# martinsbruveris/tensorflow-image-models

Measured on NVIDIA H100. Metric: images/sec fwd bs=256 224px, higher is better.
Workload: dtype bf16

## Files before the change

tensorflow-image-models_b200/csrc/common.cuh:

```cuda
#pragma once

#include <cuda.h>
#include <cuda_bf16.h>
#include <cuda_runtime.h>
#include <stdint.h>
#include <stdio.h>

#include <atomic>

#include "tfimm_b200.h"

namespace tfimm {

enum Status : int {
  kOk = TFIMM_OK,
  kInvalidArgument = TFIMM_ERR_INVALID_ARGUMENT,
  kCudaError = TFIMM_ERR_CUDA,
  kUnsupported = TFIMM_ERR_UNSUPPORTED,
};

void set_last_error(const char* fmt, ...);
int cuda_fail(cudaError_t e, const char* what);

#define TFIMM_CHECK_ARG(cond, ...)                \
// ... 277 lines not shown
__device__ __forceinline__ void st8(__nv_bfloat16* p, const float (&v)[8]) {
  uint4 a;
  a.x = pack_bf16x2(v[0], v[1]);
  a.y = pack_bf16x2(v[2], v[3]);
  a.z = pack_bf16x2(v[4], v[5]);
  a.w = pack_bf16x2(v[6], v[7]);
  *reinterpret_cast<uint4*>(p) = a;
}

__device__ __forceinline__ uint32_t smem_u32(const void* p) {
  return static_cast<uint32_t>(__cvta_generic_to_shared(p));
}

__device__ __forceinline__ bool elect_one() {
  uint32_t pred = 0;
  asm volatile(
      "{\n"
      ".reg .pred P;\n"
      "elect.sync _|P, 0xffffffff;\n"
      "selp.u32 %0, 1, 0, P;\n"
      "}\n"
      : "=r"(pred));
  return pred != 0;
}

__device__ __forceinline__ void mbar_init(uint32_t bar, uint32_t count) {
  asm volatile("mbarrier.init.shared::cta.b64 [%0], %1;" ::"r"(bar), "r"(count) : "memory");
}
__device__ __forceinline__ void fence_mbar_init() {
  asm volatile("fence.mbarrier_init.release.cluster;" ::: "memory");
}
__device__ __forceinline__ void mbar_expect_tx(uint32_t bar, uint32_t bytes) {
  asm volatile("mbarrier.arrive.expect_tx.shared::cta.b64 _, [%0], %1;" ::"r"(bar), "r"(bytes)
               : "memory");
}
__device__ __forceinline__ void mbar_arrive(uint32_t bar) {
  asm volatile("mbarrier.arrive.shared::cta.b64 _, [%0];" ::"r"(bar) : "memory");
}
__device__ __forceinline__ bool mbar_try_wait(uint32_t bar, uint32_t parity) {
  uint32_t ok;
  asm volatile(
      "{\n"
      ".reg .pred P;\n"
#ifdef TFIMM_TRYWAIT_NO_HINT
      "mbarrier.try_wait.parity.shared::cta.b64 P, [%1], %2;\n"
#else
      "mbarrier.try_wait.parity.shared::cta.b64 P, [%1], %2, %3;\n"
#endif
      "selp.u32 %0, 1, 0, P;\n"
      "}\n"
      : "=r"(ok)
      : "r"(bar), "r"(parity), "r"(1000000u)
      : "memory");
  return ok != 0;
}
__device__ __forceinline__ void mbar_wait(uint32_t bar, uint32_t parity) {
  if (mbar_try_wait(bar, parity)) return;
  const long long t0 = clock64();
  uint32_t polls = 0;
  while (!mbar_try_wait(bar, parity)) {
    if ((++polls & 255u) == 0 && clock64() - t0 > 4000000000LL) __trap();
  }
}

__device__ __forceinline__ void fence_proxy_async_smem() {
  asm volatile("fence.proxy.async.shared::cta;" ::: "memory");
}

template <int kId>
__device__ __forceinline__ void named_bar_sync(int threads) {
  asm volatile("bar.sync %0, %1;" ::"n"(kId), "r"(threads) : "memory");
}

__device__ __forceinline__ void prefetch_tmap(const void* tmap) {
  asm volatile("prefetch.tensormap [%0];" ::"l"(reinterpret_cast<uint64_t>(tmap)) : "memory");
}

__device__ __forceinline__ void tma_load_2d(uint32_t dst_smem, const void* tmap, uint32_t bar,
                                            int c0, int c1) {
  asm volatile(
      "cp.async.bulk.tensor.2d.shared::cluster.global.mbarrier::complete_tx::bytes"
      " [%0], [%1, {%3, %4}], [%2];"
      ::"r"(dst_smem), "l"(reinterpret_cast<uint64_t>(tmap)), "r"(bar), "r"(c0), "r"(c1)
      : "memory");
}
__device__ __forceinline__ void tma_store_2d(const void* tmap, uint32_t src_smem, int c0, int c1) {
  asm volatile(
      "cp.async.bulk.tensor.2d.global.shared::cta.bulk_group [%0, {%2, %3}], [%1];"
      ::"l"(reinterpret_cast<uint64_t>(tmap)), "r"(src_smem), "r"(c0), "r"(c1)
      : "memory");
}
__device__ __forceinline__ void tma_load_3d(uint32_t dst_smem, const void* tmap, uint32_t bar, int c0,
                                            int c1, int c2) {
  asm volatile(
      "cp.async.bulk.tensor.3d.shared::cluster.global.mbarrier::complete_tx::bytes"
      " [%0], [%1, {%3, %4, %5}], [%2];"
      ::"r"(dst_smem), "l"(reinterpret_cast<uint64_t>(tmap)), "r"(bar), "r"(c0), "r"(c1), "r"(c2)
      : "memory");
}
__device__ __forceinline__ void tma_load_4d(uint32_t dst_smem, const void* tmap, uint32_t bar, int c0,
                                            int c1, int c2, int c3) {
  asm volatile(
      "cp.async.bulk.tensor.4d.shared::cluster.global.mbarrier::complete_tx::bytes"
      " [%0], [%1, {%3, %4, %5, %6}], [%2];"
      ::"r"(dst_smem), "l"(reinterpret_cast<uint64_t>(tmap)), "r"(bar), "r"(c0), "r"(c1), "r"(c2), "r"(c3)
      : "memory");
}
__device__ __forceinline__ void tma_store_4d(const void* tmap, uint32_t src_smem, int c0, int c1, int c2, int c3) {
  asm volatile(
      "cp.async.bulk.tensor.4d.global.shared::cta.bulk_group [%0, {%2, %3, %4, %5}], [%1];"
      ::"l"(reinterpret_cast<uint64_t>(tmap)), "r"(src_smem), "r"(c0), "r"(c1), "r"(c2), "r"(c3)
      : "memory");
}
__device__ __forceinline__ void tma_store_3d(const void* tmap, uint32_t src_smem, int c0, int c1, int c2) {
  asm volatile(
      "cp.async.bulk.tensor.3d.global.shared::cta.bulk_group [%0, {%2, %3, %4}], [%1];"
      ::"l"(reinterpret_cast<uint64_t>(tmap)), "r"(src_smem), "r"(c0), "r"(c1), "r"(c2)
      : "memory");
}
__device__ __forceinline__ void tma_store_commit() {
  asm volatile("cp.async.bulk.commit_group;" ::: "memory");
}
template <int N>
__device__ __forceinline__ void tma_store_wait_read() {
  asm volatile("cp.async.bulk.wait_group.read %0;" ::"n"(N) : "memory");
}
template <int N>
__device__ __forceinline__ void tma_store_wait_all() {
  asm volatile("cp.async.bulk.wait_group %0;" ::"n"(N) : "memory");
}

__device__ __forceinline__ uint64_t gmma_desc_k_sw128(uint32_t smem_addr) {
  uint64_t d = 0;
  d |= (uint64_t)((smem_addr >> 4) & 0x3FFF);
  d |= (uint64_t)1 << 16;
  d |= (uint64_t)(1024 >> 4) << 32;
  d |= (uint64_t)1 << 62;
  return d;
}
__device__ __forceinline__ uint64_t gmma_desc_mn_sw128(uint32_t smem_addr) {
  uint64_t d = 0;
  d |= (uint64_t)((smem_addr >> 4) & 0x3FFF);
  d |= (uint64_t)(8192 >> 4) << 16;
  d |= (uint64_t)(1024 >> 4) << 32;
  d |= (uint64_t)1 << 62;
  return d;
}
__device__ __forceinline__ void cluster_arrive_release() {
  asm volatile("barrier.cluster.arrive.release.aligned;" ::: "memory");
}
__device__ __forceinline__ void cluster_wait_acquire() {
  asm volatile("barrier.cluster.wait.acquire.aligned;" ::: "memory");
}

__device__ __forceinline__ void wgmma_fence() { asm volatile("wgmma.fence.sync.aligned;" ::: "memory"); }
__device__ __forceinline__ void wgmma_commit() { asm volatile("wgmma.commit_group.sync.aligned;" ::: "memory"); }
template <int N>
__device__ __forceinline__ void wgmma_wait() {
  asm volatile("wgmma.wait_group.sync.aligned %0;" ::"n"(N) : "memory");
}

__device__ __forceinline__ void cp_async_16(uint32_t dst_smem, const void* src, bool valid) {
  const int sz = valid ? 16 : 0;
  asm volatile("cp.async.cg.shared.global [%0], [%1], 16, %2;" ::"r"(dst_smem), "l"(src), "r"(sz)
               : "memory");
}
__device__ __forceinline__ void cp_async_commit() { asm volatile("cp.async.commit_group;" ::: "memory"); }
template <int N>
__device__ __forceinline__ void cp_async_wait() {
  asm volatile("cp.async.wait_group %0;" ::"n"(N) : "memory");
}
__device__ __forceinline__ void ldmatrix_x4(uint32_t addr, uint32_t& r0, uint32_t& r1, uint32_t& r2,
                                            uint32_t& r3) {
  asm volatile("ldmatrix.sync.aligned.m8n8.x4.shared.b16 {%0, %1, %2, %3}, [%4];"
               : "=r"(r0), "=r"(r1), "=r"(r2), "=r"(r3)
               : "r"(addr));
}
__device__ __forceinline__ void ldmatrix_x4_trans(uint32_t addr, uint32_t& r0, uint32_t& r1,
                                                  uint32_t& r2, uint32_t& r3) {
  asm volatile("ldmatrix.sync.aligned.m8n8.x4.trans.shared.b16 {%0, %1, %2, %3}, [%4];"
               : "=r"(r0), "=r"(r1), "=r"(r2), "=r"(r3)
               : "r"(addr));
}
__device__ __forceinline__ void mma_bf16_16816(float (&d)[4], const uint32_t (&a)[4], uint32_t b0,
                                               uint32_t b1) {
  asm volatile(
      "mma.sync.aligned.m16n8k16.row.col.f32.bf16.bf16.f32 "
      "{%0, %1, %2, %3}, {%4, %5, %6, %7}, {%8, %9}, {%0, %1, %2, %3};"
      : "+f"(d[0]), "+f"(d[1]), "+f"(d[2]), "+f"(d[3])
      : "r"(a[0]), "r"(a[1]), "r"(a[2]), "r"(a[3]), "r"(b0), "r"(b1));
}

__device__ __forceinline__ uint32_t tf32_rna(float x) {
  uint32_t r;
  asm("cvt.rna.tf32.f32 %0, %1;" : "=r"(r) : "f"(x));
  return r;
}
__device__ __forceinline__ void mma_tf32_1688(float (&d)[4], const uint32_t (&a)[4], uint32_t b0, uint32_t b1) {
  asm volatile(
      "mma.sync.aligned.m16n8k8.row.col.f32.tf32.tf32.f32 "
      "{%0, %1, %2, %3}, {%4, %5, %6, %7}, {%8, %9}, {%0, %1, %2, %3};"
      : "+f"(d[0]), "+f"(d[1]), "+f"(d[2]), "+f"(d[3])
      : "r"(a[0]), "r"(a[1]), "r"(a[2]), "r"(a[3]), "r"(b0), "r"(b1));
}

#endif

}
```

tensorflow-image-models_b200/csrc/gemm_sm90.cu:

```cuda
#include <type_traits>

#include "gemm_epilogue.cuh"
#include "wgmma.cuh"

namespace tfimm {

namespace {

constexpr int kBlockM = 128;
constexpr int kRowBytes = 128;
constexpr int kConsumerThreads = 256;
constexpr int kProducerWarp = kConsumerThreads / 32;
constexpr int kNumGateWarps = 4;

enum ATransform : int {
  kANone = 0,
  kAGate = 1,
  kATf32 = 2,
};
enum GemmMode : int { kModeGemm = 0, kModeToken = 1, kModeGluCols = 2 };

template <int AX>
using OperandT = std::conditional_t<AX == kATf32, float, __nv_bfloat16>;
template <int AX>
// ... 249 lines not shown
    else if constexpr (MODE == kModeGluCols) epilogue_glu_cols<OutT, BLOCK_N>(p, acc, m_blk, n_blk, wg * 64);
    else if constexpr (STAGED)
      epilogue_staged<OutT, BLOCK_N>(p, acc, m_blk, n_blk, wg, smem_out, s_bias, s_gamma, res_bar, &tmap_c);
    else epilogue_frag<OutT, BLOCK_N>(p, acc, m_blk, n_blk, wg * 64);
  }
}

struct PersistentCfg {
  static constexpr int kBlockN = 256;
  static constexpr int kABytes = kBlockM * kRowBytes;
  static constexpr int kStageBytes = kABytes + kBlockN * kRowBytes;
  static constexpr int kStages = 3;
  static constexpr int kBoxes = 4;
  static constexpr int kOutBytes = 2 * kBoxes * kStagedBoxBytes;
  static constexpr int kVecBytes = 2 * 2 * kBlockN * 4;
  static constexpr int kNumBarriers = 2 * kStages + 2;
  static constexpr int kSmemBytes = kStages * kStageBytes + kOutBytes + kVecBytes + kNumBarriers * 8 + 1024;
};

template <typename OutT>
__global__ void __launch_bounds__(kConsumerThreads + 32, 1)
gemm_persistent_kernel(const __grid_constant__ CUtensorMap tmap_a, const __grid_constant__ CUtensorMap tmap_b,
                       const __grid_constant__ CUtensorMap tmap_c, const __grid_constant__ CUtensorMap tmap_r,
                       const GemmParams p) {
  using Cfg = PersistentCfg;
  constexpr int BN = Cfg::kBlockN, kStages = Cfg::kStages, kBlockK = 64;
  constexpr int kCols = staged_chunk_cols<OutT>(), kSpan = Cfg::kBoxes * kCols;

  extern __shared__ uint8_t smem_raw[];
  const uint32_t smem_tiles = (smem_u32(smem_raw) + 1023u) & ~1023u;
  const uint32_t smem_out = smem_tiles + kStages * Cfg::kStageBytes;
  const uint32_t smem_vec = smem_out + Cfg::kOutBytes;
  const uint32_t smem_bars = smem_vec + Cfg::kVecBytes;
  auto full_bar = [&](int s) { return smem_bars + 8u * s; };
  auto empty_bar = [&](int s) { return smem_bars + 8u * (kStages + s); };
  float* const s_vec = reinterpret_cast<float*>(smem_raw + (smem_vec - smem_u32(smem_raw)));

  const int warp_idx = threadIdx.x >> 5;
  const int lane = threadIdx.x & 31;
  if (warp_idx == kProducerWarp && lane == 0) {
    prefetch_tmap(&tmap_a);
    prefetch_tmap(&tmap_b);
    prefetch_tmap(&tmap_c);
    if (p.has_res) prefetch_tmap(&tmap_r);
    for (int s = 0; s < kStages; ++s) {
      mbar_init(full_bar(s), 1);
      mbar_init(empty_bar(s), 2);
    }
    mbar_init(smem_bars + 8u * (2 * kStages), 1);
    mbar_init(smem_bars + 8u * (2 * kStages + 1), 1);
    fence_mbar_init();
  }
  __syncthreads();

  const int num_n_tiles = (p.N + BN - 1) / BN;
  const int tiles = ((p.M + kBlockM - 1) / kBlockM) * num_n_tiles;
  const int num_k_blocks = (p.K + kBlockK - 1) / kBlockK;

  if (warp_idx == kProducerWarp) {
    if (threadIdx.x == kProducerWarp * 32) {
      int stage = 0;
      uint32_t phase = 0;
      for (int t = blockIdx.x; t < tiles; t += gridDim.x) {
        const int m_blk = t / num_n_tiles, n_blk = t % num_n_tiles;
        for (int kb = 0; kb < num_k_blocks; ++kb) {
          mbar_wait(empty_bar(stage), phase ^ 1u);
          const uint32_t sa = smem_tiles + stage * Cfg::kStageBytes;
          mbar_expect_tx(full_bar(stage), Cfg::kStageBytes);
          tma_load_2d(sa, &tmap_a, full_bar(stage), kb * kBlockK, m_blk * kBlockM);
          tma_load_2d(sa + Cfg::kABytes, &tmap_b, full_bar(stage), kb * kBlockK, n_blk * BN);
          if (++stage == kStages) { stage = 0; phase ^= 1u; }
        }
      }
    }
    return;
  }

  const int wg = warp_idx >> 2;
  const bool leader = (threadIdx.x & 127) == 0;
  const uint32_t s_wg = smem_out + (uint32_t)(wg * Cfg::kBoxes * kStagedBoxBytes);
  const uint32_t res_bar = smem_bars + 8u * (2 * kStages + wg);
  int stage = 0, prev = 0, buf = 0;
  uint32_t phase = 0, res_phase = 0;
  for (int t = blockIdx.x; t < tiles; t += gridDim.x, buf ^= 1) {
    const int m_blk = t / num_n_tiles, n_blk = t % num_n_tiles;
    const int row0 = m_blk * kBlockM + wg * 64;
    auto has_res_span = [&](int h) { return p.has_res && row0 < p.M && n_blk * BN + h * kSpan < p.N; };
    auto load_res_span = [&](int h) {
      const int col0 = n_blk * BN + h * kSpan, chunks = min(Cfg::kBoxes, (p.N - col0 + kCols - 1) / kCols);
      mbar_expect_tx(res_bar, (uint32_t)(chunks * kStagedBoxBytes));
      for (int ch = 0; ch < chunks; ++ch)
        tma_load_2d(s_wg + (uint32_t)(ch * kStagedBoxBytes), &tmap_r, res_bar, col0 + ch * kCols, row0);
    };
    float* const s_bias = s_vec + buf * 2 * BN;
    float* const s_gamma = s_bias + BN;
    const int n_own = n_blk * BN + threadIdx.x;
    const float bias_own = p.bias != nullptr && n_own < p.N ? __ldg(p.bias + n_own) : 0.f;
    const float gamma_own = p.gamma != nullptr && n_own < p.N ? __ldg(p.gamma + n_own) : 1.f;
    float acc[BN / 2];
#pragma unroll
    for (int i = 0; i < BN / 2; ++i) acc[i] = 0.f;
    for (int kb = 0; kb < num_k_blocks; ++kb) {
      mbar_wait(full_bar(stage), phase);
      const uint32_t sa = smem_tiles + stage * Cfg::kStageBytes;
      const uint64_t da = gmma_desc_k_sw128(sa + (uint32_t)wg * (64 * 128));
      const uint64_t db = gmma_desc_k_sw128(sa + Cfg::kABytes);
      wgmma_fence();
#pragma unroll
      for (int k = 0; k < 4; ++k)
        wgmma_ss<BN, false>(acc, da + (uint64_t)(2 * k), db + (uint64_t)(2 * k), (uint32_t)((kb | k) != 0));
      wgmma_commit();
      if (kb == 0) {
        s_bias[threadIdx.x] = bias_own;
        s_gamma[threadIdx.x] = gamma_own;
      }
      if (kb == num_k_blocks / 2 && leader) {
        tma_store_wait_read<0>();
        if (has_res_span(0)) load_res_span(0);
      }
      wgmma_wait<1>();
      if (kb > 0 && leader) mbar_arrive(empty_bar(prev));
      prev = stage;
      if (++stage == kStages) { stage = 0; phase ^= 1u; }
    }
    wgmma_wait<0>();
    if (leader) mbar_arrive(empty_bar(prev));

    named_bar_sync<1>(256);
    auto span = [&](auto h_const) {
      constexpr int h = decltype(h_const)::value;
      if (n_blk * BN + h * kSpan >= p.N) return;
      if constexpr (h > 0) {
        if (leader) {
          tma_store_wait_read<0>();
          if (has_res_span(h)) load_res_span(h);
        }
        warpgroup_bar_sync(wg);
      }
      if (has_res_span(h)) {
        mbar_wait(res_bar, res_phase);
        res_phase ^= 1u;
      }
      staged_apply<OutT, BN, h * kSpan, kSpan>(p, acc, s_wg, s_bias, s_gamma);
      fence_proxy_async_smem();
      warpgroup_bar_sync(wg);
      if (leader && row0 < p.M) staged_store<OutT, Cfg::kBoxes>(p, &tmap_c, s_wg, row0, n_blk * BN + h * kSpan);
    };
    span(std::integral_constant<int, 0>{});
    if constexpr (kSpan < BN) span(std::integral_constant<int, 1>{});
  }
  if (leader) tma_store_wait_read<0>();
}

int check_out(const void* C, long ldc, const void* residual, long ldr, int esize) {
  TFIMM_CHECK_ARG((reinterpret_cast<uintptr_t>(C) & 15u) == 0 && (ldc * esize) % 16 == 0,
                  "gemm: C must be 16-byte aligned with a row stride of a multiple of 16 bytes");
  TFIMM_CHECK_ARG(residual == nullptr || ((reinterpret_cast<uintptr_t>(residual) & 15u) == 0 && (ldr * esize) % 16 == 0),
                  "gemm: residual must be 16-byte aligned with a row stride of a multiple of 16 bytes");
  return kOk;
}

template <int BLOCK_N, typename OutT, int AX, int MODE, bool STAGED = false>
int launch_wgmma(const CUtensorMap& ta, const CUtensorMap& tb, const GemmParams& p, const char* what,
                 cudaStream_t stream, const CUtensorMap& tc = CUtensorMap{}, const CUtensorMap& tr = CUtensorMap{}) {
  using Cfg = GemmCfg<BLOCK_N, OutT, STAGED>;
  auto kernel = gemm_wgmma_kernel<BLOCK_N, OutT, AX, MODE, STAGED>;
  static std::atomic<unsigned long long> attr_devs{0};
  TFIMM_CUDA_OK(set_max_dynamic_smem(kernel, Cfg::kSmemBytes, attr_devs));
  const long imgs = MODE == kModeToken ? p.tk_imgs : 1;
  const long tiles = imgs * ((p.M + kBlockM - 1) / kBlockM) * ((p.N + BLOCK_N - 1) / BLOCK_N);
  kernel<<<(unsigned)tiles, gemm_threads<BLOCK_N, AX>(), Cfg::kSmemBytes, stream>>>(ta, tb, tc, tr, p);
  TFIMM_LAUNCH_OK(what);
  return kOk;
}

template <int kMaxN, typename F>
int with_block_n(int bn, const char* unsupported_fmt, F&& launch) {
  if constexpr (kMaxN >= 256) {
    if (bn == 256) return launch(std::integral_constant<int, 256>{});
  }
  if (bn == 128) return launch(std::integral_constant<int, 128>{});
  if (bn == 64) return launch(std::integral_constant<int, 64>{});
  set_last_error(unsupported_fmt, bn);
  return kInvalidArgument;
}

template <typename OutT>
int launch_persistent(const CUtensorMap& ta, const CUtensorMap& tb, const CUtensorMap& tc, const CUtensorMap& tr,
                      const GemmParams& p, cudaStream_t stream) {
  using Cfg = PersistentCfg;
  auto kernel = gemm_persistent_kernel<OutT>;
  static std::atomic<unsigned long long> attr_devs{0};
  TFIMM_CUDA_OK(set_max_dynamic_smem(kernel, Cfg::kSmemBytes, attr_devs));
  const long tiles = (long)((p.M + kBlockM - 1) / kBlockM) * ((p.N + Cfg::kBlockN - 1) / Cfg::kBlockN);
  const int grid = (int)std::min<long>(tiles, sm_count());
  kernel<<<grid, kConsumerThreads + 32, Cfg::kSmemBytes, stream>>>(ta, tb, tc, tr, p);
  TFIMM_LAUNCH_OK("gemm_persistent_kernel (bf16)");
  return kOk;
}

template <int BLOCK_N, typename OutT, int AX = kANone, int MODE = kModeGemm, bool PERSISTENT = false>
int launch_gemm(const void* A, int lda, const void* W, int ldw, const void* residual, int ldr, void* C, int ldc,
                GemmParams p, cudaStream_t stream) {
  static_assert(!PERSISTENT || (BLOCK_N == PersistentCfg::kBlockN && AX == kANone && MODE == kModeGemm),
                "the persistent instance is the plain bf16 GEMM at 256 columns");
  const int M = p.M, N = p.N, K = p.K;
  constexpr int kBlockK = block_k<AX>();
  CUtensorMap ta, tb;
  int st;
  if ((st = check_out(C, ldc, residual, ldr, (int)sizeof(OutT))) != kOk) return st;
  if ((st = make_tmap_2d(&ta, A, dtype_code<AX>(), M, K, lda, kBlockM, kBlockK, "A")) != kOk) return st;
  if ((st = make_tmap_2d(&tb, W, dtype_code<AX>(), N, K, ldw, BLOCK_N, kBlockK, "W")) != kOk) return st;
  p.c = C; p.res = residual; p.ldc = ldc; p.ldr = ldr;
  constexpr bool kStaged = AX == kANone && MODE == kModeGemm && (BLOCK_N <= 128 || PERSISTENT);
  if constexpr (kStaged) {
    if ((long)N * (long)sizeof(OutT) % 16 != 0)
      return launch_wgmma<BLOCK_N, OutT, AX, MODE>(ta, tb, p, "gemm_wgmma_kernel (bf16)", stream);
    constexpr int es = (int)sizeof(OutT), dt = es == 2 ? kBF16 : kF32;
    CUtensorMap tc, tr{};
    if ((st = make_tmap_2d(&tc, C, dt, M, N, ldc, 64, staged_chunk_cols<OutT>(), "C")) != kOk) return st;
    if (residual != nullptr &&
        (st = make_tmap_2d(&tr, residual, dt, M, N, ldr, 64, staged_chunk_cols<OutT>(), "residual")) != kOk)
      return st;
    if constexpr (PERSISTENT) return launch_persistent<OutT>(ta, tb, tc, tr, p, stream);
    else return launch_wgmma<BLOCK_N, OutT, AX, MODE, true>(ta, tb, p, "gemm_wgmma_kernel (bf16)", stream, tc, tr);
  }
  return launch_wgmma<BLOCK_N, OutT, AX, MODE>(
      ta, tb, p,
      AX == kATf32 ? "gemm_wgmma_kernel (tf32)"
                   : (MODE == kModeGluCols ? "gemm_wgmma_kernel (bf16 glu)" : "gemm_wgmma_kernel (bf16)"),
      stream);
}

template <int BLOCK_N, typename OutT>
int launch_token(const void* Wt, int ldw, const void* X, long ldx, long img_x, GemmParams p, cudaStream_t stream) {
  CUtensorMap ta, tb;
  int st;
  if ((st = check_out(p.c, p.ldc, p.res, p.ldr, (int)sizeof(OutT))) != kOk) return st;
  if ((st = make_tmap_2d(&ta, Wt, kBF16, p.M, p.K, ldw, kBlockM, 64, "token Wt")) != kOk) return st;
  {
    const uint64_t dims[3] = {(uint64_t)p.N, (uint64_t)p.K, (uint64_t)p.tk_imgs};
    const uint64_t strides[2] = {(uint64_t)ldx * 2, (uint64_t)img_x * 2};
    const uint32_t box[3] = {64u, 64u, 1u};
    if ((st = make_tmap(&tb, X, kBF16, 3, dims, strides, box, "token X")) != kOk) return st;
  }
  return launch_wgmma<BLOCK_N, OutT, kANone, kModeToken>(ta, tb, p, "gemm_wgmma_kernel (bf16 token mixing)", stream);
}

template <int BLOCK_N, typename OutT, int AX = kANone>
int launch_conv(const void* x, const void* W, int ldw, const void* residual, void* out, int B, int H, int Wd, int C,
                int Ho, int Wo, GemmParams p, cudaStream_t stream) {
  constexpr int kBlockK = block_k<AX>();
  constexpr uint64_t es = sizeof(OperandT<AX>);
  const int N = p.N, s = p.cv_stride;
  CUtensorMap ta, tb;
  int st;
  if ((st = check_out(out, N, residual, N, (int)sizeof(OutT))) != kOk) return st;
  {
    const uint64_t dims[4] = {(uint64_t)C, (uint64_t)Wd, (uint64_t)H, (uint64_t)B};
    const uint64_t strides[3] = {(uint64_t)C * es, (uint64_t)Wd * C * es, (uint64_t)H * Wd * C * es};
    const uint32_t box[4] = {(uint32_t)kBlockK, (uint32_t)(p.cv_pw * s), (uint32_t)(p.cv_ph * s), (uint32_t)p.cv_pb};
    const uint32_t estr[4] = {1u, (uint32_t)s, (uint32_t)s, 1u};
    if ((st = make_tmap(&ta, x, dtype_code<AX>(), 4, dims, strides, box, "conv input", 128, estr)) != kOk) return st;
  }
  if ((st = make_tmap_2d(&tb, W, dtype_code<AX>(), N, p.K, ldw, BLOCK_N, kBlockK, "conv weights")) != kOk) return st;
  p.c = out; p.res = residual; p.ldc = N; p.ldr = N;
  p.cv_B = B; p.cv_Ho = Ho; p.cv_Wo = Wo;
  return launch_wgmma<BLOCK_N, OutT, AX, kModeGemm>(
      ta, tb, p,
      AX == kATf32 ? "gemm_wgmma_kernel (tf32 implicit convolution)" : "gemm_wgmma_kernel (bf16 implicit convolution)",
      stream);
}

int pick_block_n(int M, int N) {
  const int sms = sm_count() > 0 ? sm_count() : 132;
  const int mt = (M + kBlockM - 1) / kBlockM;
  int best = 256;
  double best_cost = 1e30;
  for (int bn : {256, 128, 64}) {
    const int nt = (N + bn - 1) / bn;
    const long tiles = (long)mt * nt;
    const int slots = bn == 64 ? 2 * sms : sms;
    const long waves = (tiles + slots - 1) / slots;
    const double cost = (double)waves * (bn == 64 ? 2 * bn : bn) * (bn == 256 ? 1.0 : (bn == 128 ? 1.04 : 1.10));
    if (cost < best_cost) { best_cost = cost; best = bn; }
  }
  return best;
}

constexpr int kPersistent = 1;

int pick_block_n_bf16(int M, int N, int K, int out_dtype) {
  constexpr double kEpilogueK = 926.0, kPairWidth = 184.0;
  const int sms = sm_count() > 0 ? sm_count() : 132;
  const long mt = (M + kBlockM - 1) / kBlockM;
  if (N > 256 && (out_dtype == kF32 || N % 8 == 0) && mt * ((N + 255) / 256) >= sms) return kPersistent;
  const long waves128 = (mt * ((N + 127) / 128) + sms - 1) / sms;
  const long waves64 = (mt * ((N + 63) / 64) + 2 * sms - 1) / (2 * sms);
  return (double)waves64 * kPairWidth * K < (double)waves128 * 128.0 * (K + kEpilogueK) ? 64 : 128;
}

}

int gemm_bf16_skinny(const void* A, int lda, const void* W, int ldw, const float* bias, const void* residual, int ldr,
                     void* C, int ldc, int M, int N, int K, int act, cudaStream_t stream, const float* gate = nullptr,
                     int rows_per_img = 1, int imgs = 1);

int conv_setup(GemmParams& p, const float* bias, const void* residual, int B, int H, int Wd, int C, int N, int ks,
               int stride, int pad, int act, int act_post, int cblock, int& Ho, int& Wo) {
  TFIMM_CHECK_ARG(B > 0 && H > 0 && Wd > 0 && C > 0 && C % cblock == 0, "conv: C must be a multiple of %d (got %d)",
                  cblock, C);
  TFIMM_CHECK_ARG(ks >= 1 && ks <= 7 && (stride == 1 || stride == 2) && pad >= 0 && pad < ks, "conv: bad geometry");
  TFIMM_CHECK_ARG(N > 0 && N % 8 == 0, "conv: N must be a multiple of 8 (got %d)", N);
  TFIMM_CHECK_ARG(bias == nullptr || (reinterpret_cast<uintptr_t>(bias) & 15u) == 0, "conv: bias must be 16-byte aligned");
  Ho = (H + 2 * pad - ks) / stride + 1;
  Wo = (Wd + 2 * pad - ks) / stride + 1;
  TFIMM_CHECK_ARG(Ho > 0 && Wo > 0, "conv: empty output");
  p = GemmParams{};
  p.N = N; p.K = ks * ks * C;
  p.bias = bias; p.act = act; p.has_res = residual != nullptr ? 1 : 0; p.act_post = act_post;
  p.conv = 1; p.cv_cblocks = C / cblock; p.cv_ks = ks; p.cv_stride = stride; p.cv_pad = pad;
  if (Wo > 8) { p.cv_pb = 1; p.cv_ph = 8; p.cv_pw = 16; }
  else { p.cv_pb = 2; p.cv_ph = 8; p.cv_pw = 8; }
  p.cv_tiles_x = (Wo + p.cv_pw - 1) / p.cv_pw;
  p.cv_tiles_y = (Ho + p.cv_ph - 1) / p.cv_ph;
  const int tiles_b = (B + p.cv_pb - 1) / p.cv_pb;
  p.M = tiles_b * p.cv_tiles_y * p.cv_tiles_x * kBlockM;
  return kOk;
}

}

using namespace tfimm;

extern "C" {

int tfimm_b200_gemm_bf16(const void* A, int lda, const void* W, int ldw, const float* bias, const float* gamma,
                         const void* residual, int ldr, void* C, int ldc, int M, int N, int K, int act, int act_post,
                         int out_dtype, int force_block_n, void* s) {
  const cudaStream_t stream = as_stream(s);
  TFIMM_CHECK_ARG(M > 0 && N > 0 && K > 0, "gemm: M, N, K must be positive (got %d %d %d)", M, N, K);
  TFIMM_CHECK_ARG(out_dtype == kBF16 || out_dtype == kF32, "gemm: out_dtype must be bf16 or f32");
  TFIMM_CHECK_ARG(K % 8 == 0, "gemm: K must be a multiple of 8 (got %d)", K);
  TFIMM_CHECK_ARG(bias == nullptr || (reinterpret_cast<uintptr_t>(bias) & 15u) == 0, "gemm: bias must be 16-byte aligned");
  TFIMM_CHECK_ARG(gamma == nullptr || (reinterpret_cast<uintptr_t>(gamma) & 15u) == 0, "gemm: gamma must be 16-byte aligned");
  if (force_block_n == 0 && K <= 64 && out_dtype == kBF16 && gamma == nullptr && act_post == 0) {
    const int st = gemm_bf16_skinny(A, lda, W, ldw, bias, residual, ldr, C, ldc, M, N, K, act, stream);
    if (st != kUnsupported) return st;
  }
  GemmParams p{};
  p.M = M; p.N = N; p.K = K;
  p.bias = bias; p.gamma = gamma; p.act = act; p.has_res = residual != nullptr ? 1 : 0; p.act_post = act_post;
  const int bn =
      force_block_n == 2 ? 256 : (force_block_n > 0 ? force_block_n : pick_block_n_bf16(M, N, K, out_dtype));
  if (bn == kPersistent)
    return out_dtype == kBF16
               ? launch_gemm<256, __nv_bfloat16, kANone, kModeGemm, true>(A, lda, W, ldw, residual, ldr, C, ldc, p, stream)
               : launch_gemm<256, float, kANone, kModeGemm, true>(A, lda, W, ldw, residual, ldr, C, ldc, p, stream);
  return with_block_n<256>(bn, "gemm: unsupported block_n %d", [&](auto n) {
    constexpr int BN = decltype(n)::value;
    return out_dtype == kBF16 ? launch_gemm<BN, __nv_bfloat16>(A, lda, W, ldw, residual, ldr, C, ldc, p, stream)
                              : launch_gemm<BN, float>(A, lda, W, ldw, residual, ldr, C, ldc, p, stream);
  });
}

int tfimm_b200_gemm_bf16_gated(const void* A, int lda, const float* gate, int rows_per_img, int imgs, const void* W,
                               int ldw, const float* bias, const void* residual, int ldr, void* C, int ldc, int M,
                               int N, int K, int act, void* s) {
  const cudaStream_t stream = as_stream(s);
  TFIMM_CHECK_ARG(M > 0 && N > 0 && K > 0 && K % 8 == 0, "gemm_gated: need K %% 8 == 0 (got M=%d N=%d K=%d)", M, N, K);
  TFIMM_CHECK_ARG(gate != nullptr && rows_per_img > 0 && imgs > 0 && (reinterpret_cast<uintptr_t>(gate) & 15u) == 0,
                  "gemm_gated: gate [imgs][K] fp32, 16-byte aligned");
  TFIMM_CHECK_ARG(bias == nullptr || (reinterpret_cast<uintptr_t>(bias) & 15u) == 0, "gemm_gated: bias must be 16-byte aligned");
  if (K <= 64) {
    const int st = gemm_bf16_skinny(A, lda, W, ldw, bias, residual, ldr, C, ldc, M, N, K, act, stream, gate, rows_per_img,
                                    imgs);
    if (st != kUnsupported) return st;
  }
  GemmParams p{};
  p.M = M; p.N = N; p.K = K;
  p.bias = bias; p.act = act; p.has_res = residual != nullptr ? 1 : 0;
  p.a_scale = gate; p.a_rows_per_img = rows_per_img; p.a_imgs = imgs;
  return with_block_n<128>(pick_block_n(M, N) == 64 ? 64 : 128, "gemm_gated: unsupported block_n %d", [&](auto n) {
    return launch_gemm<decltype(n)::value, __nv_bfloat16, kAGate>(A, lda, W, ldw, residual, ldr, C, ldc, p, stream);
  });
}

int tfimm_b200_conv_bf16(const void* x, const void* W, int ldw, const float* bias, const void* residual, void* out,
                         int B, int H, int Wd, int C, int N, int ks, int stride, int pad, int act, int act_post,
                         int out_dtype, void* s) {
  const cudaStream_t stream = as_stream(s);
  TFIMM_CHECK_ARG(out_dtype == kBF16 || out_dtype == kF32, "conv: out_dtype must be bf16 or f32");
  GemmParams p;
  int Ho, Wo, st;
  if ((st = conv_setup(p, bias, residual, B, H, Wd, C, N, ks, stride, pad, act, act_post, 64, Ho, Wo)) != kOk)
    return st;
  return with_block_n<256>(N >= 256 ? 256 : (N >= 128 ? 128 : 64), "conv: unsupported block_n %d", [&](auto n) {
    constexpr int BN = decltype(n)::value;
    return out_dtype == kBF16 ? launch_conv<BN, __nv_bfloat16>(x, W, ldw, residual, out, B, H, Wd, C, Ho, Wo, p, stream)
                              : launch_conv<BN, float>(x, W, ldw, residual, out, B, H, Wd, C, Ho, Wo, p, stream);
  });
}

int tfimm_b200_gemm_tf32(const float* A, int lda, const float* W, int ldw, const float* bias, const float* gamma,
                         const float* residual, int ldr, float* C, int ldc, int M, int N, int K, int act, int act_post,
                         int force_block_n, void* s) {
  const cudaStream_t stream = as_stream(s);
  TFIMM_CHECK_ARG(M > 0 && N > 0 && K > 0, "gemm_tf32: M, N, K must be positive (got %d %d %d)", M, N, K);
  TFIMM_CHECK_ARG(K % 4 == 0, "gemm_tf32: K must be a multiple of 4 (got %d)", K);
  TFIMM_CHECK_ARG(bias == nullptr || (reinterpret_cast<uintptr_t>(bias) & 15u) == 0, "gemm_tf32: bias must be 16-byte aligned");
  TFIMM_CHECK_ARG(gamma == nullptr || (reinterpret_cast<uintptr_t>(gamma) & 15u) == 0,
                  "gemm_tf32: gamma must be 16-byte aligned");
  GemmParams p{};
  p.M = M; p.N = N; p.K = K;
  p.bias = bias; p.gamma = gamma; p.act = act; p.has_res = residual != nullptr ? 1 : 0; p.act_post = act_post;
  const int bn = force_block_n == 2 ? 128 : (force_block_n > 0 ? force_block_n : (pick_block_n(M, N) == 64 ? 64 : 128));
  return with_block_n<128>(bn, "gemm_tf32: unsupported block_n %d (64 or 128)", [&](auto n) {
    return launch_gemm<decltype(n)::value, float, kATf32>(A, lda, W, ldw, residual, ldr, C, ldc, p, stream);
  });
}

int tfimm_b200_conv_tf32(const float* x, const float* W, int ldw, const float* bias, const float* residual, float* out,
                         int B, int H, int Wd, int C, int N, int ks, int stride, int pad, int act, int act_post,
                         void* s) {
  const cudaStream_t stream = as_stream(s);
  GemmParams p;
  int Ho, Wo, st;
  if ((st = conv_setup(p, bias, residual, B, H, Wd, C, N, ks, stride, pad, act, act_post, 32, Ho, Wo)) != kOk)
    return st;
  return with_block_n<128>(N >= 128 ? 128 : 64, "conv: unsupported block_n %d", [&](auto n) {
    return launch_conv<decltype(n)::value, float, kATf32>(x, W, ldw, residual, out, B, H, Wd, C, Ho, Wo, p, stream);
  });
}

int tfimm_b200_token_gemm_bf16(const void* Wt, int ldw, const void* X, long ldx, long img_x, const float* bias,
                               const float* gamma, const void* residual, long ldr, long img_r, const void* mul,
                               long ld_mul, long img_mul, void* out, long ldc, long img_c, int imgs, int M, int N,
                               int K, int m_out, int act, int glu, int out_dtype, int force_block_n, void* s) {
  const cudaStream_t stream = as_stream(s);
  TFIMM_CHECK_ARG(imgs > 0 && M > 0 && N > 0 && K > 0 && m_out > 0, "token_gemm: empty shape (imgs %d M %d N %d K %d)",
                  imgs, M, N, K);
  TFIMM_CHECK_ARG(out_dtype == kBF16 || out_dtype == kF32, "token_gemm: out_dtype must be bf16 or f32");
  TFIMM_CHECK_ARG(ldw % 8 == 0 && ldw >= K && ldx % 8 == 0 && img_x % 8 == 0 && ldx >= N,
                  "token_gemm: Wt / X strides must be multiples of 8 elements");
  TFIMM_CHECK_ARG(glu ? (M % 16 == 0 && m_out <= M / 2) : m_out <= M, "token_gemm: m_out %d does not fit M %d (glu %d)",
                  m_out, M, glu);
  TFIMM_CHECK_ARG(N % 2 == 0 && (gamma == nullptr || (reinterpret_cast<uintptr_t>(gamma) & 7u) == 0),
                  "token_gemm: N must be even and gamma 8-byte aligned");
  const int es = out_dtype == kBF16 ? 2 : 4;
  TFIMM_CHECK_ARG(mul == nullptr || ((reinterpret_cast<uintptr_t>(mul) & 15u) == 0 && (ld_mul * es) % 16 == 0 &&
                                     (img_mul * es) % 16 == 0),
                  "token_gemm: mul must be 16-byte aligned with strides of multiples of 16 bytes");
  TFIMM_CHECK_ARG((img_c * es) % 16 == 0 && (residual == nullptr || (img_r * es) % 16 == 0),
                  "token_gemm: image strides must be multiples of 16 bytes");
  GemmParams p{};
  p.M = M; p.N = N; p.K = K;
  p.bias = bias; p.gamma = gamma; p.act = act; p.has_res = residual != nullptr ? 1 : 0;
  p.c = out; p.res = residual; p.ldc = ldc; p.ldr = ldr;
  p.tk_imgs = imgs; p.m_out = m_out; p.glu = glu; p.img_c = img_c; p.img_r = img_r;
  p.mul = mul; p.ld_mul = ld_mul; p.img_mul = img_mul;
  const int bn = force_block_n > 0 ? force_block_n : pick_block_n(imgs * ((M + kBlockM - 1) / kBlockM) * kBlockM, N);
  return with_block_n<256>(bn, "token_gemm: unsupported block_n %d", [&](auto n) {
    constexpr int BN = decltype(n)::value;
    return out_dtype == kBF16 ? launch_token<BN, __nv_bfloat16>(Wt, ldw, X, ldx, img_x, p, stream)
                              : launch_token<BN, float>(Wt, ldw, X, ldx, img_x, p, stream);
  });
}

int tfimm_b200_gemm_glu_bf16(const void* A, int lda, const void* W, int ldw, const float* bias, void* C, int ldc, int M,
                             int N, int K, int act, int force_block_n, void* s) {
  const cudaStream_t stream = as_stream(s);
  TFIMM_CHECK_ARG(M > 0 && N > 0 && K > 0 && K % 8 == 0 && N % 2 == 0,
                  "gemm_glu: need K %% 8 == 0 and an even N (got M=%d N=%d K=%d)", M, N, K);
  TFIMM_CHECK_ARG(bias == nullptr || (reinterpret_cast<uintptr_t>(bias) & 7u) == 0, "gemm_glu: bias must be 8-byte aligned");
  GemmParams p{};
  p.M = M; p.N = N; p.K = K;
  p.bias = bias; p.act = act;
  const int bn = force_block_n > 0 ? force_block_n : pick_block_n(M, N);
  return with_block_n<256>(bn, "gemm_glu: unsupported block_n %d", [&](auto n) {
    return launch_gemm<decltype(n)::value, __nv_bfloat16, kANone, kModeGluCols>(A, lda, W, ldw, nullptr, 0, C, ldc, p,
                                                                               stream);
  });
}

}
```

Baseline: 11650.

## Add ping-pong warp-specialized GEMM with 2-CTA cluster multicast of A tiles

Adds a persistent GEMM kernel where two consumer warpgroups alternate tiles, so one warpgroup's epilogue overlaps the other's MMA main loop. Each CTA pair in a 2-CTA cluster shares the A tile through TMA multicast and releases stages with cross-CTA mbarrier arrivals. Registers are rebalanced between producer and consumers with setmaxnreg. The heuristic picks this path for wide-N GEMMs (fp32 output, or GELU with K between 768 and 1024) that have enough tiles. This adds cluster-scheduling constraints and extra synchronization complexity.

New measurement: 11670 (median of 6 runs). No clear change (+0.2%).

```diff
diff --git a/tensorflow-image-models_b200/csrc/common.cuh b/tensorflow-image-models_b200/csrc/common.cuh
--- a/tensorflow-image-models_b200/csrc/common.cuh
+++ b/tensorflow-image-models_b200/csrc/common.cuh
@@ -453,6 +453,41 @@
 __device__ __forceinline__ void cluster_wait_acquire() {
   asm volatile("barrier.cluster.wait.acquire.aligned;" ::: "memory");
 }
+__device__ __forceinline__ uint32_t cluster_ctarank() {
+  uint32_t r;
+  asm volatile("mov.u32 %0, %%cluster_ctarank;" : "=r"(r));
+  return r;
+}
+__device__ __forceinline__ void tma_load_2d_multicast(uint32_t dst_smem, const void* tmap, uint32_t bar, int c0, int c1,
+                                                      uint16_t cta_mask) {
+  asm volatile(
+      "cp.async.bulk.tensor.2d.shared::cluster.global.mbarrier::complete_tx::bytes.multicast::cluster"
+      " [%0], [%1, {%3, %4}], [%2], %5;"
+      ::"r"(dst_smem), "l"(reinterpret_cast<uint64_t>(tmap)), "r"(bar), "r"(c0), "r"(c1), "h"(cta_mask)
+      : "memory");
+}
+__device__ __forceinline__ void mbar_arrive_cluster(uint32_t bar, uint32_t cta) {
+  asm volatile(
+      "{\n"
+      ".reg .b32 remote;\n"
+      "mapa.shared::cluster.u32 remote, %0, %1;\n"
+      "mbarrier.arrive.shared::cluster.b64 _, [remote];\n"
+      "}\n"
+      ::"r"(bar), "r"(cta)
+      : "memory");
+}
+template <int kId>
+__device__ __forceinline__ void named_bar_arrive(int threads) {
+  asm volatile("bar.arrive %0, %1;" ::"n"(kId), "r"(threads) : "memory");
+}
+template <int kRegs>
+__device__ __forceinline__ void setmaxnreg_dec() {
+  asm volatile("setmaxnreg.dec.sync.aligned.u32 %0;" ::"n"(kRegs));
+}
+template <int kRegs>
+__device__ __forceinline__ void setmaxnreg_inc() {
+  asm volatile("setmaxnreg.inc.sync.aligned.u32 %0;" ::"n"(kRegs));
+}
 
 __device__ __forceinline__ void wgmma_fence() { asm volatile("wgmma.fence.sync.aligned;" ::: "memory"); }
 __device__ __forceinline__ void wgmma_commit() { asm volatile("wgmma.commit_group.sync.aligned;" ::: "memory"); }
diff --git a/tensorflow-image-models_b200/csrc/gemm_sm90.cu b/tensorflow-image-models_b200/csrc/gemm_sm90.cu
--- a/tensorflow-image-models_b200/csrc/gemm_sm90.cu
+++ b/tensorflow-image-models_b200/csrc/gemm_sm90.cu
@@ -425,6 +425,198 @@
   if (leader) tma_store_wait_read<0>();
 }
 
+struct PingPongCfg {
+  static constexpr int kBlockN = 128;
+  static constexpr int kABytes = kBlockM * kRowBytes;
+  static constexpr int kAHalfBytes = kABytes / 2;
+  static constexpr int kStageBytes = kABytes + kBlockN * kRowBytes;
+  static constexpr int kStages = 4;
+  static constexpr int kBoxes = 4;
+  static constexpr int kOutBytes = 2 * kBoxes * kStagedBoxBytes;
+  static constexpr int kVecBytes = 2 * 2 * kBlockN * 4;
+  static constexpr int kNumBarriers = 2 * kStages + 2;
+  static constexpr int kSmemBytes = kStages * kStageBytes + kOutBytes + kVecBytes + kNumBarriers * 8 + 1024;
+  static constexpr int kThreads = kConsumerThreads + 128;
+  static constexpr int kProducerRegs = 40, kConsumerRegs = 232;
+  static_assert(kProducerRegs * 128 + kConsumerRegs * kConsumerThreads <= 65536, "register file");
+};
+
+template <typename OutT>
+__global__ void __launch_bounds__(PingPongCfg::kThreads, 1)
+gemm_pingpong_kernel(const __grid_constant__ CUtensorMap tmap_a, const __grid_constant__ CUtensorMap tmap_b,
+                     const __grid_constant__ CUtensorMap tmap_c, const __grid_constant__ CUtensorMap tmap_r,
+                     const GemmParams p) {
+  using Cfg = PingPongCfg;
+  constexpr int BN = Cfg::kBlockN, kStages = Cfg::kStages, kBlockK = 64;
+  constexpr int kCols = staged_chunk_cols<OutT>(), kSpan = 2 * kCols;
+
+  extern __shared__ uint8_t smem_raw[];
+  const uint32_t smem_tiles = (smem_u32(smem_raw) + 1023u) & ~1023u;
+  const uint32_t smem_out = smem_tiles + kStages * Cfg::kStageBytes;
+  const uint32_t smem_vec = smem_out + Cfg::kOutBytes;
+  const uint32_t smem_bars = smem_vec + Cfg::kVecBytes;
+  auto full_bar = [&](int s) { return smem_bars + 8u * s; };
+  auto empty_bar = [&](int s) { return smem_bars + 8u * (kStages + s); };
+  float* const s_vec = reinterpret_cast<float*>(smem_raw + (smem_vec - smem_u32(smem_raw)));
+
+  const int warp_idx = threadIdx.x >> 5;
+  const uint32_t rank = cluster_ctarank();
+  if (threadIdx.x == kConsumerThreads) {
+    prefetch_tmap(&tmap_a);
+    prefetch_tmap(&tmap_b);
+    prefetch_tmap(&tmap_c);
+    if (p.has_res) prefetch_tmap(&tmap_r);
+    for (int s = 0; s < kStages; ++s) {
+      mbar_init(full_bar(s), 1);
+      mbar_init(empty_bar(s), 2);
+    }
+    mbar_init(smem_bars + 8u * (2 * kStages), 1);
+    mbar_init(smem_bars + 8u * (2 * kStages + 1), 1);
+    fence_mbar_init();
+  }
+  cluster_arrive_release();
+  cluster_wait_acquire();
+
+  const int n_pairs = (p.N + 2 * BN - 1) / (2 * BN);
+  const int pairs = ((p.M + kBlockM - 1) / kBlockM) * n_pairs;
+  const int num_k_blocks = (p.K + kBlockK - 1) / kBlockK;
+  const int cluster = (int)(blockIdx.x >> 1), clusters = (int)(gridDim.x >> 1);
+
+  if (warp_idx >= kProducerWarp) {
+    setmaxnreg_dec<Cfg::kProducerRegs>();
+    if (threadIdx.x == kConsumerThreads) {
+      int stage = 0;
+      uint32_t phase = 0;
+      for (int t = cluster; t < pairs; t += clusters) {
+        const int m_blk = t / n_pairs, n_blk = 2 * (t % n_pairs) + (int)rank;
+        for (int kb = 0; kb < num_k_blocks; ++kb) {
+          mbar_wait(empty_bar(stage), phase ^ 1u);
+          const uint32_t sa = smem_tiles + stage * Cfg::kStageBytes;
+          mbar_expect_tx(full_bar(stage), Cfg::kStageBytes);
+          tma_load_2d_multicast(sa + rank * Cfg::kAHalfBytes, &tmap_a, full_bar(stage), kb * kBlockK,
+                                m_blk * kBlockM + 64 * (int)rank, 0x3);
+          tma_load_2d(sa + Cfg::kABytes, &tmap_b, full_bar(stage), kb * kBlockK, n_blk * BN);
+          if (++stage == kStages) { stage = 0; phase ^= 1u; }
+        }
+      }
+    }
+    __syncwarp();
+  } else {
+    setmaxnreg_inc<Cfg::kConsumerRegs>();
+    const int wg = warp_idx >> 2;
+    const bool leader = (threadIdx.x & 127) == 0;
+    const uint32_t s_wg = smem_out + (uint32_t)(wg * Cfg::kBoxes * kStagedBoxBytes);
+    const uint32_t res_bar = smem_bars + 8u * (2 * kStages + wg);
+    float* const s_bias = s_vec + wg * 2 * BN;
+    float* const s_gamma = s_bias + BN;
+    const int tiles = cluster < pairs ? (pairs - cluster + clusters - 1) / clusters : 0;
+    int stage = 0;
+    uint32_t phase = 0, res_phase = 0;
+    auto release = [&](int s) {
+      mbar_arrive_cluster(empty_bar(s), 0);
+      mbar_arrive_cluster(empty_bar(s), 1);
+    };
+    for (int j = 0, t = cluster; j < tiles; ++j, t += clusters) {
+      if ((j & 1) != wg) {
+        const int s = stage + num_k_blocks;
+        stage = s % kStages;
+        phase ^= (uint32_t)(s / kStages) & 1u;
+        continue;
+      }
+      const int m_blk = t / n_pairs, n_blk = 2 * (t % n_pairs) + (int)rank;
+      const int row0 = m_blk * kBlockM;
+      auto has_res_span = [&](int h) { return p.has_res && n_blk * BN + h * kSpan < p.N; };
+      auto load_res_span = [&](int h) {
+        const int col0 = n_blk * BN + h * kSpan, chunks = min(2, (p.N - col0 + kCols - 1) / kCols);
+        const int halves = p.M - row0 > 64 ? 2 : 1;
+        mbar_expect_tx(res_bar, (uint32_t)(halves * chunks * kStagedBoxBytes));
+        for (int rh = 0; rh < halves; ++rh)
+          for (int ch = 0; ch < chunks; ++ch)
+            tma_load_2d(s_wg + (uint32_t)((2 * rh + ch) * kStagedBoxBytes), &tmap_r, res_bar, col0 + ch * kCols,
+                        row0 + 64 * rh);
+      };
+      const int n_own = n_blk * BN + (threadIdx.x & 127);
+      const float bias_own = p.bias != nullptr && n_own < p.N ? __ldg(p.bias + n_own) : 0.f;
+      const float gamma_own = p.gamma != nullptr && n_own < p.N ? __ldg(p.gamma + n_own) : 1.f;
+      float acc[2][BN / 2];
+#pragma unroll
+      for (int h = 0; h < 2; ++h)
+#pragma unroll
+        for (int i = 0; i < BN / 2; ++i) acc[h][i] = 0.f;
+      if (j > 0) {
+        if (wg == 0) named_bar_sync<4>(256);
+        else named_bar_sync<5>(256);
+      }
+      int prev = 0;
+      for (int kb = 0; kb < num_k_blocks; ++kb) {
+        mbar_wait(full_bar(stage), phase);
+        const uint32_t sa = smem_tiles + stage * Cfg::kStageBytes;
+        const uint64_t da0 = gmma_desc_k_sw128(sa), da1 = gmma_desc_k_sw128(sa + Cfg::kAHalfBytes);
+        const uint64_t db = gmma_desc_k_sw128(sa + Cfg::kABytes);
+        wgmma_fence();
+#pragma unroll
+        for (int k = 0; k < 4; ++k) {
+          wgmma_ss<BN, false>(acc[0], da0 + (uint64_t)(2 * k), db + (uint64_t)(2 * k), (uint32_t)((kb | k) != 0));
+          wgmma_ss<BN, false>(acc[1], da1 + (uint64_t)(2 * k), db + (uint64_t)(2 * k), (uint32_t)((kb | k) != 0));
+        }
+        wgmma_commit();
+        if (kb == 0) {
+          s_bias[threadIdx.x & 127] = bias_own;
+          s_gamma[threadIdx.x & 127] = gamma_own;
+        }
+        if (kb == num_k_blocks / 2 && leader) {
+          tma_store_wait_read<0>();
+          if (has_res_span(0)) load_res_span(0);
+        }
+        wgmma_wait<1>();
+        if (kb > 0 && leader) release(prev);
+        prev = stage;
+        if (++stage == kStages) { stage = 0; phase ^= 1u; }
+      }
+      if (j + 1 < tiles) {
+        if (wg == 0) named_bar_arrive<5>(256);
+        else named_bar_arrive<4>(256);
+      }
+      wgmma_wait<0>();
+      if (leader) release(prev);
+
+      warpgroup_bar_sync(wg);
+#pragma unroll
+      for (int h = 0; h < BN / kSpan; ++h) {
+        if (n_blk * BN + h * kSpan >= p.N) break;
+        if (h > 0) {
+          if (leader) {
+            tma_store_wait_read<0>();
+            if (has_res_span(h)) load_res_span(h);
+          }
+          warpgroup_bar_sync(wg);
+        }
+        if (has_res_span(h)) {
+          mbar_wait(res_bar, res_phase);
+          res_phase ^= 1u;
+        }
+        if (h == 0) {
+          staged_apply<OutT, BN, 0, kSpan>(p, acc[0], s_wg, s_bias, s_gamma);
+          staged_apply<OutT, BN, 0, kSpan>(p, acc[1], s_wg + 2 * kStagedBoxBytes, s_bias, s_gamma);
+        } else {
+          staged_apply<OutT, BN, kSpan % BN, kSpan>(p, acc[0], s_wg, s_bias, s_gamma);
+          staged_apply<OutT, BN, kSpan % BN, kSpan>(p, acc[1], s_wg + 2 * kStagedBoxBytes, s_bias, s_gamma);
+        }
+        fence_proxy_async_smem();
+        warpgroup_bar_sync(wg);
+        if (leader) {
+          staged_store<OutT, 2>(p, &tmap_c, s_wg, row0, n_blk * BN + h * kSpan);
+          if (row0 + 64 < p.M)
+            staged_store<OutT, 2>(p, &tmap_c, s_wg + 2 * kStagedBoxBytes, row0 + 64, n_blk * BN + h * kSpan);
+        }
+      }
+    }
+    if (leader) tma_store_wait_read<0>();
+  }
+  cluster_arrive_release();
+  cluster_wait_acquire();
+}
+
 int check_out(const void* C, long ldc, const void* residual, long ldr, int esize) {
   TFIMM_CHECK_ARG((reinterpret_cast<uintptr_t>(C) & 15u) == 0 && (ldc * esize) % 16 == 0,
                   "gemm: C must be 16-byte aligned with a row stride of a multiple of 16 bytes");
@@ -472,30 +664,76 @@
   return kOk;
 }
 
-template <int BLOCK_N, typename OutT, int AX = kANone, int MODE = kModeGemm, bool PERSISTENT = false>
+template <typename OutT>
+int launch_pingpong(const CUtensorMap& ta, const CUtensorMap& tb, const CUtensorMap& tc, const CUtensorMap& tr,
+                    const GemmParams& p, cudaStream_t stream) {
+  using Cfg = PingPongCfg;
+  auto kernel = gemm_pingpong_kernel<OutT>;
+  static std::atomic<unsigned long long> attr_devs{0};
+  static std::atomic<int> max_clusters[64];
+  TFIMM_CUDA_OK(set_max_dynamic_smem(kernel, Cfg::kSmemBytes, attr_devs));
+  cudaLaunchConfig_t cfg{};
+  cfg.blockDim = dim3(Cfg::kThreads);
+  cfg.dynamicSmemBytes = Cfg::kSmemBytes;
+  cfg.stream = stream;
+  cudaLaunchAttribute attr[1];
+  attr[0].id = cudaLaunchAttributeClusterDimension;
+  attr[0].val.clusterDim.x = 2;
+  attr[0].val.clusterDim.y = 1;
+  attr[0].val.clusterDim.z = 1;
+  cfg.attrs = attr;
+  cfg.numAttrs = 1;
+  int dev = 0;
+  TFIMM_CUDA_OK(cudaGetDevice(&dev));
+  std::atomic<int>& fit = max_clusters[dev & 63];
+  if (fit.load(std::memory_order_relaxed) == 0) {
+    cfg.gridDim = dim3(2u * (unsigned)std::max(1, sm_count() / 2));
+    int n = 0;
+    TFIMM_CUDA_OK(cudaOccupancyMaxActiveClusters(&n, kernel, &cfg));
+    TFIMM_CHECK_ARG(n > 0, "gemm: the 2-CTA clusters of the ping-pong instance do not fit on this device");
+    fit.store(n, std::memory_order_relaxed);
+  }
+  const long pairs = (long)((p.M + kBlockM - 1) / kBlockM) * ((p.N + 2 * Cfg::kBlockN - 1) / (2 * Cfg::kBlockN));
+  cfg.gridDim = dim3(2u * (unsigned)std::min<long>(pairs, fit.load(std::memory_order_relaxed)));
+  TFIMM_CUDA_OK(cudaLaunchKernelEx(&cfg, kernel, ta, tb, tc, tr, p));
+  TFIMM_LAUNCH_OK("gemm_pingpong_kernel (bf16)");
+  return kOk;
+}
+
+constexpr int kPersistent = 1;
+constexpr int kPingPong = 3;
+
+template <int BLOCK_N, typename OutT, int AX = kANone, int MODE = kModeGemm, int WALK = 0>
 int launch_gemm(const void* A, int lda, const void* W, int ldw, const void* residual, int ldr, void* C, int ldc,
                 GemmParams p, cudaStream_t stream) {
-  static_assert(!PERSISTENT || (BLOCK_N == PersistentCfg::kBlockN && AX == kANone && MODE == kModeGemm),
-                "the persistent instance is the plain bf16 GEMM at 256 columns");
+  static_assert(WALK == 0 || (AX == kANone && MODE == kModeGemm), "the walking instances are the plain bf16 GEMM");
+  static_assert(WALK != kPersistent || BLOCK_N == PersistentCfg::kBlockN, "the persistent instance is 256 wide");
+  static_assert(WALK != kPingPong || BLOCK_N == PingPongCfg::kBlockN, "the ping-pong instance is 128 wide");
   const int M = p.M, N = p.N, K = p.K;
   constexpr int kBlockK = block_k<AX>();
   CUtensorMap ta, tb;
   int st;
   if ((st = check_out(C, ldc, residual, ldr, (int)sizeof(OutT))) != kOk) return st;
-  if ((st = make_tmap_2d(&ta, A, dtype_code<AX>(), M, K, lda, kBlockM, kBlockK, "A")) != kOk) return st;
+  constexpr uint32_t kABoxRows = WALK == kPingPong ? kBlockM / 2 : kBlockM;
+  if ((st = make_tmap_2d(&ta, A, dtype_code<AX>(), M, K, lda, kABoxRows, kBlockK, "A")) != kOk) return st;
   if ((st = make_tmap_2d(&tb, W, dtype_code<AX>(), N, K, ldw, BLOCK_N, kBlockK, "W")) != kOk) return st;
   p.c = C; p.res = residual; p.ldc = ldc; p.ldr = ldr;
-  constexpr bool kStaged = AX == kANone && MODE == kModeGemm && (BLOCK_N <= 128 || PERSISTENT);
+  constexpr bool kStaged = AX == kANone && MODE == kModeGemm && (BLOCK_N <= 128 || WALK == kPersistent);
   if constexpr (kStaged) {
-    if ((long)N * (long)sizeof(OutT) % 16 != 0)
+    if ((long)N * (long)sizeof(OutT) % 16 != 0) {
+      if constexpr (WALK == kPingPong) {
+        if ((st = make_tmap_2d(&ta, A, dtype_code<AX>(), M, K, lda, kBlockM, kBlockK, "A")) != kOk) return st;
+      }
       return launch_wgmma<BLOCK_N, OutT, AX, MODE>(ta, tb, p, "gemm_wgmma_kernel (bf16)", stream);
+    }
     constexpr int es = (int)sizeof(OutT), dt = es == 2 ? kBF16 : kF32;
     CUtensorMap tc, tr{};
     if ((st = make_tmap_2d(&tc, C, dt, M, N, ldc, 64, staged_chunk_cols<OutT>(), "C")) != kOk) return st;
     if (residual != nullptr &&
         (st = make_tmap_2d(&tr, residual, dt, M, N, ldr, 64, staged_chunk_cols<OutT>(), "residual")) != kOk)
       return st;
-    if constexpr (PERSISTENT) return launch_persistent<OutT>(ta, tb, tc, tr, p, stream);
+    if constexpr (WALK == kPersistent) return launch_persistent<OutT>(ta, tb, tc, tr, p, stream);
+    else if constexpr (WALK == kPingPong) return launch_pingpong<OutT>(ta, tb, tc, tr, p, stream);
     else return launch_wgmma<BLOCK_N, OutT, AX, MODE, true>(ta, tb, p, "gemm_wgmma_kernel (bf16)", stream, tc, tr);
   }
   return launch_wgmma<BLOCK_N, OutT, AX, MODE>(
@@ -561,12 +799,14 @@
   return best;
 }
 
-constexpr int kPersistent = 1;
-
-int pick_block_n_bf16(int M, int N, int K, int out_dtype) {
+bool pingpong_fits(int N, int out_dtype) { return ((N + 127) / 128) % 2 == 0 && (out_dtype == kF32 || N % 8 == 0); }
+
+int pick_block_n_bf16(int M, int N, int K, int out_dtype, int act) {
   constexpr double kEpilogueK = 926.0, kPairWidth = 184.0;
   const int sms = sm_count() > 0 ? sm_count() : 132;
   const long mt = (M + kBlockM - 1) / kBlockM;
+  const bool pingpong_faster = out_dtype == kF32 ? K <= 2048 : act == kActGelu && K >= 768 && K <= 1024;
+  if (pingpong_faster && N > 256 && pingpong_fits(N, out_dtype) && mt * ((N + 127) / 128) >= 2 * sms) return kPingPong;
   if (N > 256 && (out_dtype == kF32 || N % 8 == 0) && mt * ((N + 255) / 256) >= sms) return kPersistent;
   const long waves128 = (mt * ((N + 127) / 128) + sms - 1) / sms;
   const long waves64 = (mt * ((N + 63) / 64) + 2 * sms - 1) / (2 * sms);
@@ -624,12 +864,18 @@
   GemmParams p{};
   p.M = M; p.N = N; p.K = K;
   p.bias = bias; p.gamma = gamma; p.act = act; p.has_res = residual != nullptr ? 1 : 0; p.act_post = act_post;
-  const int bn =
-      force_block_n == 2 ? 256 : (force_block_n > 0 ? force_block_n : pick_block_n_bf16(M, N, K, out_dtype));
+  int bn = force_block_n == 2 ? 256 : (force_block_n > 0 ? force_block_n : pick_block_n_bf16(M, N, K, out_dtype, act));
+  if (bn == kPingPong && (N + 127) / 128 % 2 != 0) bn = pick_block_n_bf16(M, N, K, out_dtype, act);
   if (bn == kPersistent)
     return out_dtype == kBF16
-               ? launch_gemm<256, __nv_bfloat16, kANone, kModeGemm, true>(A, lda, W, ldw, residual, ldr, C, ldc, p, stream)
-               : launch_gemm<256, float, kANone, kModeGemm, true>(A, lda, W, ldw, residual, ldr, C, ldc, p, stream);
+               ? launch_gemm<256, __nv_bfloat16, kANone, kModeGemm, kPersistent>(A, lda, W, ldw, residual, ldr, C, ldc,
+                                                                                  p, stream)
+               : launch_gemm<256, float, kANone, kModeGemm, kPersistent>(A, lda, W, ldw, residual, ldr, C, ldc, p, stream);
+  if (bn == kPingPong)
+    return out_dtype == kBF16
+               ? launch_gemm<128, __nv_bfloat16, kANone, kModeGemm, kPingPong>(A, lda, W, ldw, residual, ldr, C, ldc, p,
+                                                                                stream)
+               : launch_gemm<128, float, kANone, kModeGemm, kPingPong>(A, lda, W, ldw, residual, ldr, C, ldc, p, stream);
   return with_block_n<256>(bn, "gemm: unsupported block_n %d", [&](auto n) {
     constexpr int BN = decltype(n)::value;
     return out_dtype == kBF16 ? launch_gemm<BN, __nv_bfloat16>(A, lda, W, ldw, residual, ldr, C, ldc, p, stream)
```
